# catid/siamese

Hardware: AMD Instinct MI355X
Metric: device-resident GB/s encode+decode, 1400B pkts @20% loss; % HBM peak (higher is better)
Workload: dtype u8

## Files before the change

### siamese_amd/csrc/decoder.cpp

```cpp
#include "decoder.h"
#include "frames.h"

#include <algorithm>
#include <atomic>
#include <cstdio>
#include <cstdlib>
#include <cstring>
#include <x86intrin.h>

namespace sgpu {

namespace {

inline unsigned popcount_range(uint64_t bits, unsigned begin, unsigned end)
{
    if (begin >= end)
        return 0;
    uint64_t mask = (end >= 64 ? ~0ULL : ((1ULL << end) - 1)) & ~((1ULL << begin) - 1);
    return (unsigned)__builtin_popcountll(bits & mask);
}

inline unsigned first_clear(uint64_t bits, unsigned from)
{
    if (from >= 64)
// ... 2222 lines not shown

bool DecoderCore::pivoted_ge(unsigned pivot)
{
    const unsigned columns = matCols_;
    const unsigned rows = matRows_;
    unsigned j = pivot + 1;
    bool resume = true;
    for (; pivot < columns; ++pivot) {
        if (!resume)
            j = pivot;
        resume = false;
        bool found = false;
        for (; j < rows; ++j) {
            const unsigned rj = pivots_[j];
            const uint8_t* ge = mrow(rj);
            const uint8_t val = ge[pivot];
            if (val == 0)
                continue;
            if (pivot != j)
                std::swap(pivots_[pivot], pivots_[j]);
            rows_[rj].used = true;
            const unsigned end = rows_[rj].columnCount;
            if (pivot >= columns - 1)
                return true;
            for (unsigned k = pivot + 1; k < rows; ++k) {
                const unsigned rk = pivots_[k];
                if (eliminate_row(ge, mrow(rk), pivot, end, val) && rows_[rk].columnCount < end)
                    rows_[rk].columnCount = end;
            }
            found = true;
            break;
        }
        if (!found) {
            geResume_ = pivot;
            return false;
        }
    }
    return true;
}


bool DecoderCore::eliminate_original_data()
{
    ++scanEpoch_;
    const unsigned rows = region_.recoveryCount;
    bool haveRun = false;
    unsigned runStart = 0, runCount = 0, runEnd = 0, runBytes = 0, runSumStart = 0;
    uint32_t fresh = 0;
    WinEntry sums[kRowSums];
    uint32_t clip[kRowSums];
    uint32_t present = 0;
    bool tableStale = true;
    uint64_t tableVersion = 0;
    for (unsigned ri = 0; ri < rows; ++ri) {
        if (!rows_[ri].used)
            continue;
        RecPacket* rec = rows_[ri].rec;
        const RowMeta m = rec->meta;
        const unsigned es = rec->elementStart;
        const unsigned ee = rec->elementEnd;
        const unsigned rb = rec->bytes;

        if (m.sumCount <= kCauchyThreshold) {
            prog_.lc_begin(rec->buf.addr(), rb, rb);
            for (unsigned j = es; j < ee; ++j) {
                const DecSlot& o = slot(j);
                if (o.bytes == 0)
                    continue;
                const uint8_t y = m.row == 0 ? 1 : cauchy_element(m.row - 1, o.column % kCauchyMaxColumns);
                prog_.lc_term(o.buf.addr(), std::min(o.bytes, rb), y);
                account_elim(std::min(o.bytes, rb));
            }
            prog_.lc_end();
            continue;
        }

        const bool sameRun = haveRun && m.columnStart == runStart && m.sumCount == runCount &&
                             ee == runEnd && rb == runBytes && recoveredColumns_.empty();
        unsigned sumElementStart = column_to_element(m.columnStart);
        if (!sameRun) {
            if (m.columnStart != sumColumnStart_ || m.sumCount < sumColumnCount_) {
                if (sumElementStart >= count_)
                    return false;
                reset_sums(sumElementStart);
                sumColumnStart_ = m.columnStart;
            } else {
                if (sumElementStart >= count_)
                    sumElementStart = 0;
                if (!start_sums(sumElementStart, rb))
                    return false;
            }
            sumColumnCount_ = m.sumCount;
            haveRun = true;
            runStart = m.columnStart;
            runCount = m.sumCount;
            runEnd = ee;
            runBytes = rb;
            fresh = 0;
            tableStale = true;
            runSumStart = sumElementStart;
        }

        windowLo_ = std::min(es, runSumStart);
        const RowSelect& sel = row_select(m.row);
        const uint32_t want = sel.mask[0] | sel.mask[1];
        uint32_t need = want & ~fresh;
        if (need)
            tableStale = true;
        for (; need; need &= need - 1) {
            const unsigned k = (unsigned)__builtin_ctz(need);
            if (get_sum(k / kSums, k % kSums, ee).bytes > 0)
                materialize(k / kSums, k % kSums);
        }
        fresh |= want;
        if (tableStale) {
            tableStale = false;
            tableVersion = Program::next_table_version();
            present = 0;
            for (unsigned k = 0; k < kRowSums; ++k) {
                const DevSum& d = sum(k / kSums, k % kSums).d;
                WinEntry& t = sums[k];
                t.src = d.buf.addr();
                t.len = d.bytes;
                t.column = 0;
                if (d.bytes > 0)
                    present |= 1u << k;
                clip[k] = std::min(d.bytes, rb);
            }
        }
        uint64_t opBytes = rb;
        for (uint32_t b = sel.mask[0] & present; b; b &= b - 1)
            opBytes += clip[__builtin_ctz(b)];
        for (uint32_t b = sel.mask[1] & present; b; b &= b - 1)
            opBytes += clip[__builtin_ctz(b)];
        const uint32_t mask[2] = {sel.mask[0] & present, sel.mask[1] & present};
        cover(windowLo_, ee);
        prog_.rows_row(sums, rec->buf.addr(), rb, rb, row_value(m.row), mask[0], mask[1], m.row,
                       m.ldpcCount, es, ee, nullptr, 0, tableVersion);
        account_elim(opBytes);
    }
    prog_.rows_seal();
    return !disabled_;
}


SiameseResult DecoderCore::solve_and_substitute()
{
    unsigned slot = 0;
    if (!solve_plan(0, &slot)) {
        disabled_ = true;
        return Siamese_Disabled;
    }
    return solve_publish(slot);
}

bool DecoderCore::solve_plan(uint32_t gateWord, unsigned* slotOut)
{
    const unsigned m = region_.lostCount;
    std::vector<RecPacket*>& pr = scratchRec_;
    std::vector<unsigned>& len = scratchLen_;
    pr.resize(m);
    len.resize(m);
    for (unsigned i = 0; i < m; ++i) {
        pr[i] = rows_[pivots_[i]].rec;
        len[i] = pr[i]->bytes;
    }
    SolveRow* desc = nullptr;
    uint8_t* coefOut = nullptr;
    prog_.solve_reserve(m, &desc, &coefOut);
    for (unsigned i = 0; i < m; ++i) {
        std::memset(&desc[i], 0, sizeof(SolveRow));
        desc[i].initBytes = len[i];
    }
    uint64_t lowerOpBytes = 0;
    bool equal = true;
    for (unsigned i = 1; i < m && equal; ++i)
        equal = len[i] == len[0];
    if (equal) {
        if (!gateWord) {
            uint64_t nz = 0;
            for (unsigned j = 1; j < m; ++j)
                nz += gf_count_nonzero(mrow(pivots_[j]), j);
            lowerOpBytes = nz * (m ? len[0] : 0);
        }
        for (unsigned i = 0; i + 1 < m; ++i)
            desc[i].lowerLen = len[i];
    } else {
        for (unsigned i = 0; i + 1 < m; ++i) {
            desc[i].lowerLen = len[i];
            for (unsigned j = i + 1; j < m; ++j) {
                if (mrow(pivots_[j])[i] == 0)
                    continue;
                lowerOpBytes += len[i];
// ... 536 lines not shown
```

### siamese_amd/csrc/encoder.cpp

```cpp
#include "encoder.h"
#include "frames.h"

#include <algorithm>
#include <atomic>
#include <cstdio>
#include <cstdlib>
#include <cstring>

namespace sgpu {

namespace {

constexpr unsigned kSlotCauses = 6;
const char* const kSlotCauseNames[kSlotCauses] = {"add", "length", "stride", "stamp", "arq", "other"};
struct SlotCounts
{
    const bool on = std::getenv("SIAMESE_AMD_SLOT_COUNTS") != nullptr;
    std::atomic<uint64_t> encoders{0}, uniform{0}, writes{0};
    std::atomic<uint64_t> demote[kSlotCauses] = {};
    ~SlotCounts()
    {
        if (!on)
            return;
        std::fprintf(stderr, "slot counts: encoders %llu enc_uniform %llu enc_slot_writes %llu",
// ... 879 lines not shown
    stats_[SiameseEncoderStats_RecoveryCount]++;
    stats_[SiameseEncoderStats_RecoveryBytes] += out.bytes;
}

SiameseResult EncoderCore::encode(EncodeOut& out)
{
    lastRowSiamese_ = false;
    if (dead())
        return Siamese_Disabled;
    if (count_ == 0) {
        out.bytes = 0;
        return Siamese_NeedMoreData;
    }
    if (firstUnremoved_ >= kRemoveThreshold)
        remove_elements();

    const unsigned inFlight = unacked();
    if (inFlight == 1)
        return single_row(out);

    const unsigned sumWidthBound = count_ - sumStart_ + sumErased_;
    if (sumEnd_ <= sumStart_ || sumWidthBound >= kMaxPacketsInFlight) {
        if (inFlight <= kCauchyThreshold)
            return cauchy_row(out);
        reset_sums(firstUnremoved_);
    } else if (inFlight <= kSumResetThreshold || sumWidthBound <= kCauchyThreshold) {
        sumEnd_ = sumStart_;
        return cauchy_row(out);
    }

    const unsigned row = nextRow_;
    if (++nextRow_ >= kRowValuePeriod)
        nextRow_ = 0;
    return siamese_row(out, row);
}

SiameseResult EncoderCore::encode_range(EncodeOut* out, unsigned count, unsigned* produced)
{
    for (DevBuf& b : recoveryHeld_)
        eng_->release(b);
    recoveryHeld_.clear();
    return encode_range_more(out, count, produced);
}

SiameseResult EncoderCore::encode_range_more(EncodeOut* out, unsigned count, unsigned* produced)
{
    *produced = 0;
    std::vector<DevBuf> held;
    held.swap(recoveryHeld_);
    SiameseResult r = Siamese_Success;
    bool siamese = false;
    uint64_t opAcc = 0, outAcc = 0;
    for (unsigned k = 0; k < count; ++k) {
        if (k > 0 || !held.empty() || *produced) {
            held.push_back(recovery_);
            recovery_ = DevBuf();
        }
        if (siamese) {
            if (dead()) {
                r = Siamese_Disabled;
                break;
            }
            const unsigned row = nextRow_;
            if (++nextRow_ >= kRowValuePeriod)
                nextRow_ = 0;
            recovery_ = eng_->alloc(longest_ + kMaxFooterBytes);
            if (!recovery_) {
                disabled_ = true;
                r = Siamese_Disabled;
                break;
            }
            uint64_t ob = 0;
            r = siamese_row_body(out[k], row, &ob);
            if (r != Siamese_Success)
                break;
            opAcc += ob;
            outAcc += out[k].bytes;
        } else {
            r = encode(out[k]);
            if (r != Siamese_Success)
                break;
            siamese = lastRowSiamese_;
        }
        ++*produced;
    }
    eng_->account(opAcc, outAcc);
    recoveryHeld_.swap(held);
    return r;
}

SiameseResult EncoderCore::single_row(EncodeOut& out)
{
    const SlotView o = peek(firstUnremoved_);
    if (!ensure_recovery(o.bytes + kMaxFooterBytes))
        return Siamese_Disabled;
    prog_.lc_begin(recovery_.addr(), o.bytes, 0);
    prog_.lc_term(o.addr(), o.bytes, 1);
    prog_.lc_end();
    write_length_prefix(o.bytes - o.header, out.head);
    RowMeta m;
    m.sumCount = 1;
    m.ldpcCount = 1;
    m.columnStart = o.column;
    m.row = 0;
    finish_row(out, m, o.bytes);
    return Siamese_Success;
// ... 70 lines not shown
        get_sum(k / kSums, k % kSums, count_);
        if (dead())
            return Siamese_Disabled;
    }
    staleSums_ &= ~want;
    if (sumTableStale_ || sumClipBytes_ != recoveryBytes) {
        sumTableStale_ = false;
        sumTableVersion_ = Program::next_table_version();
        sumPresent_ = 0;
        sumClipBytes_ = recoveryBytes;
        for (unsigned k = 0; k < kRowSums; ++k) {
            const DevSum& d = lanes_[k / kSums].sum[k % kSums];
            WinEntry& t = sumTable_[k];
            t.src = d.buf.addr();
            t.len = d.bytes;
            t.column = 0;
            if (d.bytes > 0)
                sumPresent_ |= 1u << k;
            sumClip_[k] = std::min(d.bytes, recoveryBytes);
        }
    }
    const uint32_t mask[2] = {sel.mask[0] & sumPresent_, sel.mask[1] & sumPresent_};
    uint64_t opBytes = recoveryBytes;
    for (unsigned h = 0; h < 2; ++h)
        for (uint32_t b = mask[h]; b; b &= b - 1)
            opBytes += sumClip_[__builtin_ctz(b)];
    sumEnd_ = count_;

    RowMeta m;
    m.sumCount = sumEnd_ - sumStart_ + sumErased_;
    m.ldpcCount = unacked();
    m.columnStart = sumColumnStart_;
    m.row = row;
    const unsigned footerBytes = write_footer(m, out.footer);

    const unsigned start = firstUnremoved_;
    const unsigned n = sumEnd_ - start;

    cover(std::min(start, sumStart_), sumEnd_);
    prog_.rows_row(sumTable_, recovery_.addr(), recoveryBytes, 0, row_value(row), mask[0], mask[1], row,
                   n, start, count_, out.footer, footerBytes, sumTableVersion_);

    out.meta = m;
    out.footerBytes = footerBytes;
    out.buf = recovery_;
    out.bytes = recoveryBytes + footerBytes;
    stats_[SiameseEncoderStats_RecoveryCount]++;
    stats_[SiameseEncoderStats_RecoveryBytes] += out.bytes;
    lastRowSiamese_ = true;
    *opBytesOut = opBytes;
    return Siamese_Success;
}

SiameseResult EncoderCore::stats(uint64_t* out, unsigned count)
{
    if (count > SiameseEncoderStats_Count)
        count = SiameseEncoderStats_Count;
    uint64_t mem = recovery_.cap;
    for (auto& sw : subwindows_) {
        mem += sw->slab.buf.cap;
        if (sw->clean)
            continue;
        for (EncSlot& s : sw->slot)
            if (!s.inSlab)
                mem += s.buf.cap;
    }
    for (Lane& l : lanes_)
        for (DevSum& s : l.sum)
            mem += s.buf.cap;
    stats_[SiameseEncoderStats_MemoryUsed] = mem;
    for (unsigned i = 0; i < count; ++i)
        out[i] = stats_[i];
    return Siamese_Success;
}

}
```

### siamese_amd/csrc/encoder.h

```cpp
#pragma once

#include "arq.h"
#include "codedef.h"
#include "engine.h"
#include "objpool.h"
#include "../../include/siamese.h"

#include <memory>
#include <vector>

namespace sgpu {

struct EncSlot
{
    DevBuf buf;
    bool inSlab = false;
    unsigned bytes = 0;
    unsigned column = 0;
    unsigned header = 0;
    uint32_t lastSend = 0;
    std::unique_ptr<std::vector<uint8_t>> hostp;
    std::vector<uint8_t>& host()
    {
        if (!hostp)
// ... 148 lines not shown
        }
        return v;
    }
    void demote(EncSubwindow* sw, DemoteCause cause);
    static uint64_t run_bits(unsigned bit, unsigned m) { return (m >= 64 ? ~0ull : (1ull << m) - 1) << bit; }
    bool uniform_takes(EncSubwindow* sw, unsigned element, unsigned m, unsigned need, unsigned h, unsigned column,
                       uint32_t stamp);
    void add_uniform(EncSubwindow* sw, unsigned element, unsigned m, unsigned need, unsigned h, unsigned bytes,
                     unsigned column, uint32_t stamp);
    void release_subwindow(EncSubwindow* sw);
#ifdef SGPU_SLOT_CHECK
    void slot_check(const EncSubwindow* sw, const char* where) const;
    struct AddExpect
    {
        unsigned nextColumn, longest, laneLongest[kLanes], count;
        uint32_t stale;
        uint64_t oc, ob;
        size_t subs;
    };
    AddExpect slot_check_add(EncSubwindow* sw, unsigned element, unsigned m, const unsigned* lens, unsigned fixedBytes,
                             uint32_t stamp);
    void slot_check_added(const AddExpect& x) const;
    [[noreturn]] static void slot_check_failed(const char* where, const char* what, unsigned bit);
#endif
    unsigned column_to_element(unsigned c) const { return column_sub(c, columnStart_); }
    unsigned element_to_column(unsigned e) const { return column_add(e, columnStart_); }
    unsigned next_lane_element(unsigned element, unsigned lane) const
    {
        unsigned e = element - (element % kLanes) + lane;
        return e < element ? e + kLanes : e;
    }
    unsigned unacked() const { return count_ - firstUnremoved_; }
    unsigned take_element();
    bool place(unsigned element, unsigned need);
    void fill_slot(EncSlot& s, unsigned column, unsigned header, unsigned dataBytes, uint32_t stamp);
    void release_slot(EncSlot& s)
    {
        if (!s.inSlab)
            eng_->release(s.buf);
        s.buf = DevBuf();
        s.inSlab = false;
    }
    void start_window(unsigned column);
    void reset_sums(unsigned elementStart);
    void remove_elements();
    DevSum& get_sum(unsigned lane, unsigned sumIndex, unsigned elementEnd);
    void cover(unsigned lo, unsigned hi);
    bool grow_sum(DevSum& s, unsigned bytes);

    SiameseResult single_row(EncodeOut& out);
    SiameseResult cauchy_row(EncodeOut& out);
    SiameseResult siamese_row(EncodeOut& out, unsigned row);
    SiameseResult siamese_row_body(EncodeOut& out, unsigned row, uint64_t* opBytes);
    bool ensure_recovery(unsigned bytes);
    void finish_row(EncodeOut& out, const RowMeta& meta, unsigned payloadBytes,
                    bool footerWritten = false);
    void update_rto();
    SiameseResult retransmit_slot(EncSlot& s, SiameseOriginalPacket& out);
    AckState ack_;

    Engine* eng_;
    Program prog_;
    bool mirror_;
    bool disabled_ = false;

    std::vector<EncSubwindowPtr> subwindows_;
    struct SubwindowTable
    {
        std::vector<EncSubwindowPtr> v;
        std::vector<DevBuf> held;
    };
    unsigned nextColumn_ = 0;
    unsigned count_ = 0;
    unsigned columnStart_ = 0;
    unsigned longest_ = 0;
    unsigned firstUnremoved_ = 0;
    unsigned sumStart_ = 0, sumEnd_ = 0, sumColumnStart_ = 0, sumErased_ = 0;

    struct Lane
    {
        unsigned next[kSums];
        DevSum sum[kSums];
        unsigned longest = 0;
    } lanes_[kLanes];

    static constexpr uint32_t kAllSums = (1u << kRowSums) - 1;
    uint32_t staleSums_ = kAllSums;
    WinEntry sumTable_[kRowSums];
    uint32_t sumPresent_ = 0;
    bool sumTableStale_ = true;
    uint64_t sumTableVersion_ = 0;
    uint32_t sumClip_[kRowSums] = {};
    unsigned sumClipBytes_ = ~0u;
    bool lastRowSiamese_ = false;

    DevBuf recovery_;
    std::vector<DevBuf> recoveryHeld_;
    unsigned nextRow_ = 0;
    unsigned nextParityColumn_ = 0;
    unsigned nextCauchyRow_ = 0;

    uint64_t stats_[SiameseEncoderStats_Count] = {};

    unsigned uniformEntered_ = 0, slotWrites_ = 0;
    unsigned demotions_[kDemoteCauses] = {};
};
// ... 3 lines not shown
```

### siamese_amd/csrc/engine.cpp

```cpp
#include "engine.h"

#include <pthread.h>
#include "backend.h"
#include "codedef.h"
#include "pool.h"

#include <algorithm>
#include <chrono>
#include <cmath>
#include <cstdio>
#include <cstddef>
#include <cstdlib>
#include <cstring>

#ifndef SGPU_EXEC_LPT
#define SGPU_EXEC_LPT 1
#endif
#ifndef SGPU_EXEC_GROUPS
#define SGPU_EXEC_GROUPS 256
#endif

namespace sgpu {

void EngineStats::add(const EngineStats& o)
// ... 56 lines not shown
    }
    return new ProgramBody;
}

void ProgramBody::put(ProgramBody* b)
{
    b->clear();
    std::lock_guard<std::mutex> g(g_bodyMu);
    if (g_bodies.size() < (1u << 15))
        g_bodies.push_back(b);
    else
        delete b;
}

void ProgramBody::clear()
{
    for (size_t k = 0; k < nsegs; ++k)
        segs[k].clear();
    nsegs = 0;
    resultWords = 0;
    nsolves = 0;
    nges = 0;
    callbacks.clear();
    keep.clear();
    rb.open = false;
    rb.win.clear();
    rb.updates.clear();
    rb.rows.clear();
    copies.clear();
    lcb.clear();
    ndeliver = 0;
    nframe = 0;
    frameLit.clear();
    frameLitRefs.clear();
    nrelay = 0;
    npackjob = npack = 0;
    nconcatjob = nconcat = 0;
    gateOpen = false;
}

void ProgramBody::new_segment()
{
    rows_close();
    if (nsegs == segs.size())
        segs.emplace_back();
    segs[nsegs++].clear();
}

void ProgramBody::rows_open(uint32_t base, bool keepWindow)
{
    rows_close();
    if (nsegs == 0)
        new_segment();
    rb.open = true;
    rb.haveSums = false;
    rb.sumsVersion = 0;
    rb.readMask = 0;
    rb.cutMax = 0;
    rb.versioned = false;
    if (!keepWindow) {
        rb.base = base;
        rb.win.clear();
    }
    rb.updates.clear();
    for (int& u : rb.updateOf)
        u = -1;
    rb.rows.clear();
    rb.maxExtent = 0;
}

namespace {
inline bool overlaps(uint64_t a, uint64_t an, uint64_t b, uint64_t bn) { return a < b + bn && b < a + an; }
inline uint64_t lane_span(uint32_t n) { return ((uint64_t)n + 15) & ~(uint64_t)15; }
}

void ProgramBody::lc_seal()
{
    if (lcb.items.empty())
        return;
    Segment& s = segs[nsegs - 1];
    if (lcb.items.size() == 1) {
        const LcItem& it = lcb.items[0];
        GfOp op;
        std::memset(&op, 0, sizeof(op));
        op.dst = it.dst;
        op.n = it.n;
        op.valid = it.valid;
        op.kind = OP_LINCOMB;
        op.mix = it.mixLit & 0xff;
        op.termBegin = (uint32_t)s.terms.size();
        op.termCount = it.termCount;
        s.ops.push_back(op);
        s.terms.insert(s.terms.end(), lcb.terms.begin(), lcb.terms.end());
        const uint32_t litLen = (it.mixLit >> 8) & 0xff;
        if (litLen) {
            GfOp lo;
            std::memset(&lo, 0, sizeof(lo));
            lo.dst = it.dst;
            lo.n = it.litOffset;
            lo.valid = litLen;
            lo.kind = OP_LITERAL;
            std::memcpy(lo.lit, it.lit, litLen);
            s.ops.push_back(lo);
        }
        lcb.clear();
        return;
    }
    const uint32_t itemWords = (uint32_t)lcb.items.size() * kLcWords;
    for (LcItem& it : lcb.items)
        it.termStart += itemWords;
    GfOp op;
    std::memset(&op, 0, sizeof(op));
    op.kind = OP_LINCOMBS;
    op.n = (uint32_t)lcb.items.size();
    op.termBegin = (uint32_t)(s.rowsData.size() / 16);
    op.termCount = itemWords + (uint32_t)lcb.terms.size();
    s.ops.push_back(op);
    const size_t at = s.rowsData.size();
    s.rowsData.resize(at + (size_t)op.termCount * 16);
    std::memcpy(s.rowsData.data() + at, lcb.items.data(), lcb.items.size() * sizeof(LcItem));
    std::memcpy(s.rowsData.data() + at + lcb.items.size() * sizeof(LcItem), lcb.terms.data(),
// ... 497 lines not shown
    return b.win.data() + (end - b.base);
}

void Program::rows_update(unsigned k, uint64_t dst, uint32_t n, uint32_t valid, unsigned s,
                          uint32_t fromElement, uint32_t toElement)
{
    ProgramBody::RowsBuild& b = b_->rb;
    if (b.readMask >> k & 1) {
        const WinEntry& seen = b.sums[k];
        if (seen.src != dst || valid < seen.len || toElement - fromElement > kVersionMaxSpan ||
            b.rows.size() >= kVersionRows)
            rows_open(b.base, true);
        else
            b.versioned = true;
    }
    const uint32_t from = fromElement - b.base, to = toElement - b.base;
    int& ui = b.updateOf[k];
    if (ui >= 0) {
        SumUpdate& u = b.updates[ui];
        const uint64_t d = ((uint64_t)u.dstHi << 32) | u.dstLo;
        if (d == dst && (u.to == from || from == to)) {
            if (from != to)
                u.to = to;
            if (n > u.n)
                u.n = n;
            if (n > b.maxExtent)
                b.maxExtent = n;
            return;
        }
        rows_open(b.base, true);
    }
    SumUpdate u;
    std::memset(&u, 0, sizeof(u));
    u.dstLo = (uint32_t)dst;
    u.dstHi = (uint32_t)(dst >> 32);
    u.n = n;
    u.valid = valid < n ? valid : n;
    u.s = s;
    u.from = from;
    u.to = to < from ? from : to;
    u.sum = k;
    b.updateOf[k] = (int)b.updates.size();
    b.updates.push_back(u);
    if (n > b.maxExtent)
        b.maxExtent = n;
}

uint64_t Program::next_table_version()
{
    static std::atomic<uint64_t> next{1};
    return next.fetch_add(1, std::memory_order_relaxed);
}

void Program::rows_row(const WinEntry* sums, uint64_t dst, uint32_t n, uint32_t valid, uint8_t mix,
                       uint32_t mask0, uint32_t mask1, unsigned row, uint32_t ldpcN,
                       uint32_t ldpcFirst, uint32_t cutoff, const uint8_t* lit, uint32_t litLen,
                       uint64_t sumsVersion)
{
    ProgramBody::RowsBuild& b = b_->rb;
    const bool unchanged = sumsVersion != 0 && b.haveSums && b.sumsVersion == sumsVersion;
    bool same = true;
    if (b.haveSums && !unchanged)
        for (uint32_t r = b.readMask; r; r &= r - 1) {
            const unsigned k = (unsigned)__builtin_ctz(r);
            if (std::memcmp(&b.sums[k], &sums[k], sizeof(WinEntry)) != 0) {
                same = false;
                break;
            }
        }
    if (!same || cutoff < b.cutMax || (b.versioned && b.rows.size() >= kVersionRows))
        rows_open(b.base, true);
    b.cutMax = std::max(b.cutMax, cutoff);
    if (!(unchanged && b.haveSums))
        std::memcpy(b.sums, sums, sizeof(b.sums));
    b.haveSums = true;
    b.sumsVersion = sumsVersion;
    RowItem r;
    std::memset(&r, 0, sizeof(r));
    r.dst = dst;
    r.n = n;
    r.valid = valid < n ? valid : n;
    r.mask0 = mask0 | (litLen << 24);
    r.mask1 = mask1 | ((uint32_t)mix << 24);
    r.row = row;
    r.ldpcN = ldpcN;
    r.ldpcOff = ldpcFirst - b.base;
    r.cutoff = cutoff - b.base;
    if (litLen)
        std::memcpy(r.lit, lit, litLen);
    b.rows.push_back(r);
    b.readMask |= mask0 | mask1;
    if (n + litLen > b.maxExtent)
        b.maxExtent = n + litLen;
}

void Program::copy(uint64_t dst, uint64_t src, uint32_t len)
{
    if (len == 0)
        return;
    touch();
    if (b_->copies.empty()) {
        b_->rows_close();
        if (b_->nsegs == 0)
            b_->new_segment();
    }
    CopyItem c;
    std::memset(&c, 0, sizeof(c));
    c.dst = dst;
    c.src = src;
    c.len = len;
    b_->copies.push_back(c);
    ProgramBody::Segment& g = b_->segs[b_->nsegs - 1];
    if (len > g.maxExtent)
        g.maxExtent = len;
}

void Program::deliver(uint64_t src, uint32_t cap, uint64_t dst, uint64_t lenOut, uint64_t stride)
{
    touch();
    DeliverItem it;
    it.src = src;
    it.dst = dst;
    it.lenOut = lenOut;
    it.cap = cap;
    it.stride16 = (uint32_t)(stride >> 4);
    if (b_->ndeliver == b_->delivers.size())
        b_->delivers.emplace_back();
    b_->delivers[b_->ndeliver++] = it;
}

void Program::frame(uint64_t src, uint32_t bytes, const uint8_t* hdr, uint32_t hdrLen, uint64_t dst,
                    uint64_t lenOut, uint64_t stride, uint32_t lenBase)
{
    touch();
    FrameItem it;
    it.src = src;
    it.dst = dst;
    it.lenOut = lenOut;
    it.bytes = bytes;
    it.stride16 = (uint32_t)(stride >> 4);
    std::memset(it.hdr, 0, sizeof(it.hdr));
    std::memcpy(it.hdr, hdr, hdrLen);
    it.hdrLen = (uint8_t)hdrLen;
    it.lenBase = lenBase;
    if (b_->nframe == b_->frames.size())
        b_->frames.emplace_back();
    b_->frames[b_->nframe++] = it;
}
// ... 252 lines not shown
        if (cls < depot_.size()) {
            auto& mags = depot_[cls];
            for (size_t k = mags.size(); k-- > 0;) {
                if (mags[k].ticket > done)
                    continue;
                list.swap(mags[k].bufs);
                mags.erase(mags.begin() + (long)k);
                if (!list.empty())
                    return true;
                break;
            }
        }
    }
    if (cap > kRegionBytes / 4) {
        uint8_t* p = carve_region(cap);
        if (!p)
            return false;
        list.push_back(p);
        return true;
    }
    const size_t want = std::max<size_t>(1, std::min<size_t>(kMagazine, kRefillBytes / cap));
    for (size_t k = 0; k < want; ++k) {
        if (s.bumpLeft < cap) {
            if (k > 0)
                break;
            uint8_t* r = carve_region(kRegionBytes);
            if (!r)
                return false;
            s.bump = r;
            s.bumpLeft = kRegionBytes;
        }
        list.push_back(s.bump);
        s.bump += cap;
        s.bumpLeft -= cap;
    }
    return true;
}

DevBuf Engine::alloc(uint32_t bytes)
{
    DevBuf b;
    const uint32_t cap = round_cap(bytes);
    Shard& s = shard();
    const size_t cls = cap_class(cap);
    if (cls >= s.freeLists.size())
        s.freeLists.resize(cls + 1);
    if (s.freeLists[cls].empty() && !refill(s, cls, cap))
        return DevBuf();
    b.ptr = s.freeLists[cls].back();
    s.freeLists[cls].pop_back();
    b.cap = cap;
    s.inUse += cap;
    return b;
}


DevBuf Engine::slab_slot(Slab& sl, unsigned bit, uint32_t need, bool* failed)
{
    *failed = false;
    if (!sl.buf) {
        static_assert(kSubwindow == 64, "slab_stride's slot count");
        const uint32_t stride = slab_stride(need);
        if (!stride)
            return DevBuf();
        sl.buf = alloc(stride * kSubwindow);
        if (!sl.buf) {
            *failed = true;
            return DevBuf();
        }
        sl.stride = stride;
        sl.used = 0;
    }
    if (need > sl.stride || (sl.used >> bit & 1u))
        return DevBuf();
    sl.used |= 1ull << bit;
    DevBuf b;
    b.ptr = sl.buf.ptr + (size_t)bit * sl.stride;
    b.cap = sl.stride;
    return b;
}

void Engine::release(DevBuf& b)
{
    if (b.ptr) {
        Shard& s = shard();
        const size_t cls = cap_class(b.cap);
        if (cls >= s.q.released.size())
            s.q.released.resize(cls + 1);
        s.q.released[cls].push_back(b.ptr);
        s.inUse -= b.cap;
    }
    b = DevBuf();
}

void Engine::download(void* hostDst, uint64_t devSrc, uint32_t bytes)
{
    if (bytes)
        shard().q.downloads.push_back(Shard::Download{hostDst, devSrc, bytes});
}

void Engine::stage_host_ingest(const DevBuf& dst, const void* data, uint32_t bytes,
                               const uint8_t* hdr, uint32_t hdrLen)
{
    Shard& s = shard();
    const size_t off = (s.q.hostStage.size() + 15) & ~(size_t)15;
    s.q.hostStage.resize(off + hdrLen + bytes);
// ... 1799 lines not shown
```

### siamese_amd/csrc/engine.h

```cpp
#pragma once

#include "ops.h"

#include <atomic>
#include <condition_variable>
#include <cstdint>
#include <cstdio>
#include <cstdlib>
#include <deque>
#include <functional>
#include <memory>
#include <mutex>
#include <pthread.h>
#include <shared_mutex>
#include <thread>
#include <vector>

namespace sgpu {

class InstanceLock
{
public:
    InstanceLock() = default;
    InstanceLock(const InstanceLock&) = delete;
// ... 147 lines not shown
using Completion = std::function<void(const uint32_t* results)>;

struct ProgramBody
{
    struct Segment
    {
        std::vector<GfOp> ops;
        std::vector<GfTerm> terms;
        std::vector<uint8_t> rowsData;
        uint32_t rowsWords = 0;
        uint32_t maxExtent = 0;
        struct Wide
        {
            uint32_t op;
            uint32_t entry;
            uint32_t n, row, N, off;
        };
        std::vector<Wide> wide;
        uint32_t wideItems = 0;
        uint64_t wideBytes = 0;
        struct Gate
        {
            uint32_t opBegin, opEnd, word;
        };
        std::vector<Gate> gates;
        void clear()
        {
            ops.clear();
            terms.clear();
            rowsData.clear();
            rowsWords = 0;
            maxExtent = 0;
            wide.clear();
            wideItems = 0;
            wideBytes = 0;
            gates.clear();
        }
    };
    struct RowsBuild
    {
        bool open = false;
        bool haveSums = false;
        uint64_t sumsVersion = 0;
        WinEntry sums[kRowSums];
        uint32_t readMask = 0;
        uint32_t cutMax = 0;
        bool versioned = false;
        uint32_t base = 0;
        std::vector<WinEntry> win;
        std::vector<SumUpdate> updates;
        int updateOf[kRowSums];
        std::vector<RowItem> rows;
        uint32_t maxExtent = 0;
    };
    struct PendingSolve
    {
        SolveDesc desc;
        std::vector<SolveRow> rows;
        std::vector<uint8_t> coef;
        mutable uint32_t asmRow = 0, asmCoef = 0;
    };
    struct PendingGe
    {
        uint16_t rows = 0, cols = 0;
        uint32_t pickLen = 0;
        uint32_t result = 0;
        bool chained = false;
        uint32_t solve = ~0u;
        std::vector<uint8_t> in;
    };

    int group = 0;
    uint32_t resultWords = 0;
    size_t nsegs = 0;
    std::vector<Segment> segs;
    std::vector<PendingSolve> solves;
    size_t nsolves = 0;
    std::vector<PendingGe> ges;
    uint32_t nges = 0;
    uint32_t ndeliver = 0;
    uint32_t nframe = 0;
    uint32_t nrelay = 0;
    std::vector<Completion> callbacks;
    std::vector<std::shared_ptr<void>> keep;
    RowsBuild rb;
    bool gateOpen = false;
    size_t gateSeg = 0;
    uint32_t gateOp = 0, gateWord = 0;
    std::vector<CopyItem> copies;
    struct LcBuild
    {
        std::vector<LcItem> items;
        std::vector<GfTerm> terms;
        struct Span
        {
            uint64_t lo, hi;
        };
        std::vector<Span> writes, reads;
        void clear()
        {
            items.clear();
            terms.clear();
            writes.clear();
            reads.clear();
        }
    } lcb;
// ... 53 lines not shown
            len = op.n;
        if (len == 0 || coeff == 0)
            return;
        GfTerm t;
        t.src = src;
        t.len = len;
        t.coeff = coeff;
        t.acc = acc;
        t.pad = 0;
        s.terms.push_back(t);
        ++op.termCount;
    }
    void lc_end();

    void add_mem(uint64_t dst, uint64_t src, uint32_t n);
    void muladd_mem(uint64_t dst, uint8_t y, uint64_t src, uint32_t n);
    void mul_mem(uint64_t dst, uint64_t src, uint8_t y, uint32_t n);
    void zero(uint64_t dst, uint32_t n);

    void literal(uint64_t dst, uint32_t offset, const uint8_t* bytes, uint32_t len);

    void ingest_host(const DevBuf& dst, const void* data, uint32_t bytes, const uint8_t* hdr,
                     uint32_t hdrLen);
    void ingest_device(const DevBuf& dst, uint64_t src, uint32_t bytes, const uint8_t* hdr,
                       uint32_t hdrLen);
    void ingest_run(uint64_t dst, uint32_t dstStride, uint64_t src, uint32_t srcStride, uint32_t count,
                    uint32_t bytes, const uint8_t* hdr, uint32_t hdrLen);

    uint32_t solve(const std::vector<SolveRow>& rows, const uint8_t* coef, uint32_t maxBytes);
    void solve_reserve(unsigned m, SolveRow** rows, uint8_t** coef);
    uint32_t solve_commit(uint32_t maxBytes, uint32_t gateWord = 0);

    uint8_t* ge_job(unsigned rows, unsigned cols, unsigned pickLen, uint32_t* resultWord, bool chained = false);
    void gate_begin(uint32_t word);
    uint32_t gate_end();

    void on_complete(Completion fn);
    void on_complete(std::shared_ptr<void> keep, Completion fn);
    void drop_callbacks()
    {
        if (b_) {
            b_->callbacks.clear();
            b_->keep.clear();
        }
    }

    WinEntry* rows_window(uint32_t lo, uint32_t hi, uint32_t* from);
    void rows_update(unsigned sumIndex, uint64_t dst, uint32_t n, uint32_t valid, unsigned s,
                     uint32_t fromElement, uint32_t toElement);
    void rows_row(const WinEntry* sums, uint64_t dst, uint32_t n, uint32_t valid, uint8_t mix,
                  uint32_t mask0, uint32_t mask1, unsigned row, uint32_t ldpcN,
                  uint32_t ldpcFirst, uint32_t cutoff, const uint8_t* lit = nullptr, uint32_t litLen = 0,
                  uint64_t sumsVersion = 0);
    static uint64_t next_table_version();
    void rows_seal()
    {
        if (b_)
            b_->rows_close();
    }

    void copy(uint64_t dst, uint64_t src, uint32_t len);

    void deliver(uint64_t src, uint32_t cap, uint64_t dst, uint64_t lenOut, uint64_t stride);

    void frame(uint64_t src, uint32_t bytes, const uint8_t* hdr, uint32_t hdrLen, uint64_t dst, uint64_t lenOut,
               uint64_t stride, uint32_t lenBase = 0);
    void frame_literal(const uint8_t* data, uint32_t bytes, const uint8_t* hdr, uint32_t hdrLen, uint64_t dst,
                       uint64_t lenOut, uint64_t stride);

    void relay(uint64_t src, uint32_t cap, uint32_t flow, uint32_t packetNum, uint64_t dst, uint64_t lenOut,
               uint64_t stride);

    void pack(const PackItem* items, uint32_t count, uint64_t rows, uint64_t stride, uint32_t maxRows, uint64_t lens,
              uint64_t info);

    void concat(const ConcatItem* items, uint32_t count, uint32_t total, uint64_t dst, uint32_t capacity,
                uint64_t offsets, uint64_t info);

    bool empty() const { return !b_ || b_->empty(); }

private:
    friend class Engine;
    void touch()
    {
        if (!shard_)
            attach();
    }
    void attach();
    void rows_open(uint32_t base, bool keepWindow) { b_->rows_open(base, keepWindow); }

    Engine* eng_;
    int group_;
    Shard* shard_ = nullptr;
    ProgramBody* b_ = nullptr;
};

struct EngineStats
{
    uint64_t flushes = 0, launches = 0, ops = 0, terms = 0, solves = 0, ingests = 0;
    uint64_t uploadBytes = 0;
    uint64_t refOpBytes = 0, outBytes = 0;
    uint64_t solveBytes = 0;
    uint64_t ldpcBytes = 0;
    uint64_t assembleNs = 0, waitNs = 0, completeNs = 0, reclaimNs = 0;
    uint64_t execLaunches = 0;
    uint64_t execUniqueBytes = 0;
    uint64_t geJobs = 0, geChained = 0, geRetried = 0;
    uint64_t geChainedWide = 0;
    uint64_t delivers = 0;
    uint64_t frames = 0;
    uint64_t scans = 0;
    uint64_t relays = 0;

    void add(const EngineStats& o);
};

class Engine
{
public:
    static Engine* global();
    ~Engine();

    bool init(int device, const char** err);
    bool ready() const { return ready_; }

    DevBuf alloc(uint32_t bytes);
    void release(DevBuf& b);
    DevBuf slab_slot(Slab& sl, unsigned bit, uint32_t need, bool* failed);
    void slab_release(Slab& sl)
    {
        release(sl.buf);
        sl.stride = 0;
        sl.used = 0;
    }
    uint64_t bytes_in_use() const;
    uint64_t arena_bytes() const { return arenaBytes_.load(std::memory_order_relaxed); }
    bool reserve(size_t bytes);

    void download(void* hostDst, uint64_t devSrc, uint32_t bytes);

    uint64_t enqueue();
    bool wait(uint64_t ticket);
    bool done(uint64_t ticket)
    {
        std::lock_guard<std::mutex> g(qMu_);
        return doneTicket_ >= ticket;
    }
    uint64_t last_ticket() const { return nextTicket_.load(std::memory_order_acquire); }
    bool flush();
    bool sync() { return wait(nextTicket_.load(std::memory_order_acquire)); }
    bool flush_and_sync(InstanceLock* detach = nullptr);
    bool failed() const { return failed_.load(std::memory_order_relaxed); }
    bool pending() const;

    bool gather(unsigned count, const void* const* srcs, const unsigned* bytes, void* hostOut);
    bool gather_completed(unsigned count, const void* const* srcs, const unsigned* bytes, void* pinnedOut);
    int64_t gather_async(unsigned count, const void* const* srcs, const unsigned* bytes, void* pinnedOut);
    int64_t gather_async_framed(unsigned count, const void* const* srcs, const unsigned* bytes,
                                const uint8_t* hdrs, const unsigned* hdrLens, void* pinnedOut);
    int64_t scan_rows_async(const void* rows, uint64_t stride, const uint32_t* lens, unsigned count,
                            void* pinnedOut)
    {
        return rows_async(rows, stride, lens, count, 0, pinnedOut);
    }
    int64_t walk_rows_async(const void* rows, uint64_t stride, const uint32_t* lens, unsigned count,
                            unsigned maxFrames, void* pinnedOut)
    {
        return rows_async(rows, stride, lens, count, maxFrames, pinnedOut);
    }
    int64_t duplex_rows_async(const void* rows, uint64_t stride, const uint32_t* lens, unsigned count,
                              unsigned maxFrames, unsigned ackSlots, unsigned ackBytes, void* pinnedOut)
    {
        return rows_async(rows, stride, lens, count, maxFrames, pinnedOut, ackSlots, ackBytes);
    }
    int64_t dense_rows_async(const void* rows, uint64_t stride, const uint32_t* lens, unsigned count,
                             unsigned maxFrames, unsigned maxRecords, void* pinnedOut)
    {
        return rows_async(rows, stride, lens, count, maxFrames, pinnedOut, 0, 0, maxRecords);
    }
// ... 191 lines not shown
```

Baseline: 4238.

## Batch consecutive Siamese recovery rows into single row-run submissions

```diff
diff --git a/siamese_amd/csrc/decoder.cpp b/siamese_amd/csrc/decoder.cpp
--- a/siamese_amd/csrc/decoder.cpp
+++ b/siamese_amd/csrc/decoder.cpp
@@ -2298,9 +2298,34 @@
     uint32_t present = 0;
     bool tableStale = true;
     uint64_t tableVersion = 0;
+    thread_local std::vector<Program::RowSpec> pend;
+    pend.clear();
+    uint64_t pendBytes = 0;
+    bool afterSiamese = false;
+    unsigned runEs = 0, runLdpc = 0;
+    auto flush_run = [&] {
+        if (pend.empty())
+            return;
+        Program::RowRun run;
+        run.sums = sums;
+        run.n = runBytes;
+        run.valid = runBytes;
+        run.ldpcN = runLdpc;
+        run.ldpcFirst = runEs;
+        run.cutoff = runEnd;
+        run.sumsVersion = tableVersion;
+        cover(windowLo_, runEnd);
+        prog_.rows_run(run, pend.data(), (unsigned)pend.size());
+        account_elim(pendBytes);
+        pend.clear();
+        pendBytes = 0;
+    };
     for (unsigned ri = 0; ri < rows; ++ri) {
-        if (!rows_[ri].used)
+        if (!rows_[ri].used) {
+            flush_run();
+            afterSiamese = false;
             continue;
+        }
         RecPacket* rec = rows_[ri].rec;
         const RowMeta m = rec->meta;
         const unsigned es = rec->elementStart;
@@ -2308,6 +2333,8 @@
         const unsigned rb = rec->bytes;
 
         if (m.sumCount <= kCauchyThreshold) {
+            flush_run();
+            afterSiamese = false;
             prog_.lc_begin(rec->buf.addr(), rb, rb);
             for (unsigned j = es; j < ee; ++j) {
                 const DecSlot& o = slot(j);
@@ -2323,6 +2350,25 @@
 
         const bool sameRun = haveRun && m.columnStart == runStart && m.sumCount == runCount &&
                              ee == runEnd && rb == runBytes && recoveredColumns_.empty();
+        const RowSelect& sel = row_select(m.row);
+        const uint32_t want = sel.mask[0] | sel.mask[1];
+        if (sameRun && afterSiamese && es == runEs && m.ldpcCount == runLdpc && !tableStale && !(want & ~fresh)) {
+            const uint32_t mask[2] = {sel.mask[0] & present, sel.mask[1] & present};
+            pendBytes += rb;
+            for (unsigned h = 0; h < 2; ++h)
+                for (uint32_t b = mask[h]; b; b &= b - 1)
+                    pendBytes += clip[__builtin_ctz(b)];
+            Program::RowSpec s;
+            std::memset(&s, 0, sizeof(s));
+            s.dst = rec->buf.addr();
+            s.row = m.row;
+            s.mask0 = mask[0];
+            s.mask1 = mask[1];
+            s.mix = row_value(m.row);
+            pend.push_back(s);
+            continue;
+        }
+        flush_run();
         unsigned sumElementStart = column_to_element(m.columnStart);
         if (!sameRun) {
             if (m.columnStart != sumColumnStart_ || m.sumCount < sumColumnCount_) {
@@ -2348,8 +2394,6 @@
         }
 
         windowLo_ = std::min(es, runSumStart);
-        const RowSelect& sel = row_select(m.row);
-        const uint32_t want = sel.mask[0] | sel.mask[1];
         uint32_t need = want & ~fresh;
         if (need)
             tableStale = true;
@@ -2384,7 +2428,11 @@
         prog_.rows_row(sums, rec->buf.addr(), rb, rb, row_value(m.row), mask[0], mask[1], m.row,
                        m.ldpcCount, es, ee, nullptr, 0, tableVersion);
         account_elim(opBytes);
-    }
+        afterSiamese = true;
+        runEs = es;
+        runLdpc = m.ldpcCount;
+    }
+    flush_run();
     prog_.rows_seal();
     return !disabled_;
 }
diff --git a/siamese_amd/csrc/encoder.cpp b/siamese_amd/csrc/encoder.cpp
--- a/siamese_amd/csrc/encoder.cpp
+++ b/siamese_amd/csrc/encoder.cpp
@@ -955,6 +955,19 @@
     bool siamese = false;
     uint64_t opAcc = 0, outAcc = 0;
     for (unsigned k = 0; k < count; ++k) {
+        if (siamese) {
+            const unsigned len = run_rows(count - k);
+            if (len > 1) {
+                const unsigned made = siamese_run(out + k, len, held, &opAcc, &outAcc);
+                *produced += made;
+                if (made < len) {
+                    r = Siamese_Disabled;
+                    break;
+                }
+                k += len - 1;
+                continue;
+            }
+        }
         if (k > 0 || !held.empty() || *produced) {
             held.push_back(recovery_);
             recovery_ = DevBuf();
@@ -1131,6 +1144,110 @@
     return Siamese_Success;
 }
 
+unsigned EncoderCore::run_rows(unsigned most) const
+{
+    if (sumTableStale_ || sumClipBytes_ != longest_)
+        return 0;
+    if (!staleSums_)
+        return most;
+    unsigned len = 0;
+    for (unsigned row = nextRow_; len < most; ++len) {
+        const RowSelect& sel = row_select(row);
+        if ((sel.mask[0] | sel.mask[1]) & staleSums_)
+            break;
+        if (++row >= kRowValuePeriod)
+            row = 0;
+    }
+    return len;
+}
+
+unsigned EncoderCore::siamese_run(EncodeOut* out, unsigned count, std::vector<DevBuf>& held, uint64_t* opAcc,
+                                  uint64_t* outAcc)
+{
+    if (dead()) {
+        held.push_back(recovery_);
+        recovery_ = DevBuf();
+        return 0;
+    }
+    thread_local std::vector<DevBuf> runBufs_;
+    thread_local std::vector<Program::RowSpec> runSpec_;
+    runBufs_.resize(count);
+    const unsigned got = eng_->alloc_run(longest_ + kMaxFooterBytes, runBufs_.data(), count);
+
+    const unsigned recoveryBytes = longest_;
+    RowMeta m;
+    m.sumCount = count_ - sumStart_ + sumErased_;
+    m.ldpcCount = unacked();
+    m.columnStart = sumColumnStart_;
+    m.row = 0;
+    uint8_t footer[kMaxFooterBytes] = {};
+    const unsigned footerBytes = write_footer(m, footer);
+    const bool footerRow = m.sumCount > 1;
+    const unsigned start = firstUnremoved_;
+    const unsigned bytes = recoveryBytes + footerBytes;
+
+    if (got) {
+        sumEnd_ = count_;
+        cover(std::min(start, sumStart_), sumEnd_);
+        runSpec_.resize(got);
+    }
+    uint64_t opBytes = 0;
+    for (unsigned k = 0; k < got; ++k) {
+        held.push_back(recovery_);
+        recovery_ = runBufs_[k];
+        const unsigned row = nextRow_;
+        if (++nextRow_ >= kRowValuePeriod)
+            nextRow_ = 0;
+        const RowSelect& sel = row_select(row);
+        const uint32_t mask[2] = {sel.mask[0] & sumPresent_, sel.mask[1] & sumPresent_};
+        opBytes += recoveryBytes;
+        for (unsigned h = 0; h < 2; ++h)
+            for (uint32_t b = mask[h]; b; b &= b - 1)
+                opBytes += sumClip_[__builtin_ctz(b)];
+        if (footerRow)
+            footer[0] = (uint8_t)row;
+        Program::RowSpec& s = runSpec_[k];
+        s.dst = recovery_.addr();
+        s.row = row;
+        s.mask0 = mask[0];
+        s.mask1 = mask[1];
+        s.mix = row_value(row);
+        s.litLen = (uint8_t)footerBytes;
+        std::memcpy(s.lit, footer, sizeof(s.lit));
+        EncodeOut& o = out[k];
+        m.row = row;
+        o.meta = m;
+        std::memcpy(o.footer, footer, footerBytes);
+        o.footerBytes = footerBytes;
+        o.buf = recovery_;
+        o.bytes = bytes;
+    }
+    if (got) {
+        Program::RowRun run;
+        run.sums = sumTable_;
+        run.n = recoveryBytes;
+        run.valid = 0;
+        run.ldpcN = sumEnd_ - start;
+        run.ldpcFirst = start;
+        run.cutoff = count_;
+        run.sumsVersion = sumTableVersion_;
+        prog_.rows_run(run, runSpec_.data(), got);
+        stats_[SiameseEncoderStats_RecoveryCount] += got;
+        stats_[SiameseEncoderStats_RecoveryBytes] += (uint64_t)got * bytes;
+        lastRowSiamese_ = true;
+        *opAcc += opBytes;
+        *outAcc += (uint64_t)got * bytes;
+    }
+    if (got < count) {
+        held.push_back(recovery_);
+        recovery_ = DevBuf();
+        if (++nextRow_ >= kRowValuePeriod)
+            nextRow_ = 0;
+        disabled_ = true;
+    }
+    return got;
+}
+
 SiameseResult EncoderCore::stats(uint64_t* out, unsigned count)
 {
     if (count > SiameseEncoderStats_Count)
diff --git a/siamese_amd/csrc/encoder.h b/siamese_amd/csrc/encoder.h
--- a/siamese_amd/csrc/encoder.h
+++ b/siamese_amd/csrc/encoder.h
@@ -224,6 +224,9 @@
     SiameseResult cauchy_row(EncodeOut& out);
     SiameseResult siamese_row(EncodeOut& out, unsigned row);
     SiameseResult siamese_row_body(EncodeOut& out, unsigned row, uint64_t* opBytes);
+    unsigned run_rows(unsigned most) const;
+    unsigned siamese_run(EncodeOut* out, unsigned count, std::vector<DevBuf>& held, uint64_t* opAcc,
+                         uint64_t* outAcc);
     bool ensure_recovery(unsigned bytes);
     void finish_row(EncodeOut& out, const RowMeta& meta, unsigned payloadBytes,
                     bool footerWritten = false);
diff --git a/siamese_amd/csrc/engine.cpp b/siamese_amd/csrc/engine.cpp
--- a/siamese_amd/csrc/engine.cpp
+++ b/siamese_amd/csrc/engine.cpp
@@ -132,21 +132,26 @@
     rows_close();
     if (nsegs == 0)
         new_segment();
-    rb.open = true;
-    rb.haveSums = false;
-    rb.sumsVersion = 0;
-    rb.readMask = 0;
-    rb.cutMax = 0;
-    rb.versioned = false;
+    rb.restart(base, keepWindow);
+}
+
+void ProgramBody::RowsBuild::restart(uint32_t newBase, bool keepWindow)
+{
+    open = true;
+    haveSums = false;
+    sumsVersion = 0;
+    readMask = 0;
+    cutMax = 0;
+    versioned = false;
     if (!keepWindow) {
-        rb.base = base;
-        rb.win.clear();
-    }
-    rb.updates.clear();
-    for (int& u : rb.updateOf)
+        base = newBase;
+        win.clear();
+    }
+    updates.clear();
+    for (int& u : updateOf)
         u = -1;
-    rb.rows.clear();
-    rb.maxExtent = 0;
+    rows.clear();
+    maxExtent = 0;
 }
 
 namespace {
@@ -750,12 +755,13 @@
     return next.fetch_add(1, std::memory_order_relaxed);
 }
 
-void Program::rows_row(const WinEntry* sums, uint64_t dst, uint32_t n, uint32_t valid, uint8_t mix,
-                       uint32_t mask0, uint32_t mask1, unsigned row, uint32_t ldpcN,
-                       uint32_t ldpcFirst, uint32_t cutoff, const uint8_t* lit, uint32_t litLen,
-                       uint64_t sumsVersion)
-{
-    ProgramBody::RowsBuild& b = b_->rb;
+namespace {
+
+template <class Open>
+inline void row_into(ProgramBody::RowsBuild& b, Open&& open, const WinEntry* sums, uint64_t dst, uint32_t n,
+                     uint32_t valid, uint8_t mix, uint32_t mask0, uint32_t mask1, unsigned row, uint32_t ldpcN,
+                     uint32_t ldpcFirst, uint32_t cutoff, const uint8_t* lit, uint32_t litLen, uint64_t sumsVersion)
+{
     const bool unchanged = sumsVersion != 0 && b.haveSums && b.sumsVersion == sumsVersion;
     bool same = true;
     if (b.haveSums && !unchanged)
@@ -767,7 +773,7 @@
             }
         }
     if (!same || cutoff < b.cutMax || (b.versioned && b.rows.size() >= kVersionRows))
-        rows_open(b.base, true);
+        open();
     b.cutMax = std::max(b.cutMax, cutoff);
     if (!(unchanged && b.haveSums))
         std::memcpy(b.sums, sums, sizeof(b.sums));
@@ -792,6 +798,150 @@
         b.maxExtent = n + litLen;
 }
 
+#ifdef SGPU_ROWRUN_CHECK
+struct RowRunCheck
+{
+    struct Seen
+    {
+        bool haveSums, versioned;
+        WinEntry sums[kRowSums];
+        uint32_t readMask, cutMax, maxExtent;
+        std::vector<RowItem> rows;
+    };
+    static Seen see(const ProgramBody::RowsBuild& b)
+    {
+        Seen s;
+        s.haveSums = b.haveSums;
+        s.versioned = b.versioned;
+        std::memcpy(s.sums, b.sums, sizeof(s.sums));
+        s.readMask = b.readMask;
+        s.cutMax = b.cutMax;
+        s.maxExtent = b.maxExtent;
+        s.rows = b.rows;
+        return s;
+    }
+    static bool equal(const Seen& a, const Seen& b)
+    {
+        return a.haveSums == b.haveSums && a.versioned == b.versioned &&
+               (!a.haveSums || std::memcmp(a.sums, b.sums, sizeof(a.sums)) == 0) && a.readMask == b.readMask &&
+               a.cutMax == b.cutMax && a.maxExtent == b.maxExtent && a.rows.size() == b.rows.size() &&
+               (a.rows.empty() || std::memcmp(a.rows.data(), b.rows.data(), a.rows.size() * sizeof(RowItem)) == 0);
+    }
+    ProgramBody::RowsBuild shadow;
+    std::vector<Seen> want, got;
+
+    RowRunCheck(const ProgramBody::RowsBuild& b, const Program::RowRun& run, const Program::RowSpec* rows,
+                unsigned count)
+        : shadow(b)
+    {
+        for (unsigned k = 0; k < count; ++k) {
+            const Program::RowSpec& s = rows[k];
+            row_into(
+                shadow,
+                [&] {
+                    want.push_back(see(shadow));
+                    shadow.restart(shadow.base, true);
+                },
+                run.sums, s.dst, run.n, run.valid, s.mix, s.mask0, s.mask1, s.row, run.ldpcN, run.ldpcFirst,
+                run.cutoff, s.lit, s.litLen, run.sumsVersion);
+        }
+    }
+    void closing(const ProgramBody::RowsBuild& b) { got.push_back(see(b)); }
+    void done(const ProgramBody::RowsBuild& b)
+    {
+        want.push_back(see(shadow));
+        got.push_back(see(b));
+        bool ok = want.size() == got.size() && shadow.sumsVersion == b.sumsVersion && shadow.base == b.base;
+        for (size_t k = 0; ok && k < want.size(); ++k)
+            ok = equal(want[k], got[k]);
+        if (!ok) {
+            std::fprintf(stderr, "rows_run: the run differs from its rows emitted one by one (%zu / %zu batches)\n",
+                         got.size(), want.size());
+            std::abort();
+        }
+    }
+};
+#endif
+
+}
+
+void Program::rows_row(const WinEntry* sums, uint64_t dst, uint32_t n, uint32_t valid, uint8_t mix,
+                       uint32_t mask0, uint32_t mask1, unsigned row, uint32_t ldpcN,
+                       uint32_t ldpcFirst, uint32_t cutoff, const uint8_t* lit, uint32_t litLen,
+                       uint64_t sumsVersion)
+{
+    ProgramBody::RowsBuild& b = b_->rb;
+    row_into(b, [&] { rows_open(b.base, true); }, sums, dst, n, valid, mix, mask0, mask1, row, ldpcN, ldpcFirst,
+             cutoff, lit, litLen, sumsVersion);
+}
+
+void Program::rows_run(const RowRun& run, const RowSpec* rows, unsigned count)
+{
+    if (count == 0)
+        return;
+    ProgramBody::RowsBuild& b = b_->rb;
+#ifdef SGPU_ROWRUN_CHECK
+    RowRunCheck check(b, run, rows, count);
+#define ROWRUN_CLOSING() check.closing(b)
+#else
+#define ROWRUN_CLOSING() (void)0
+#endif
+    const bool unchanged = run.sumsVersion != 0 && b.haveSums && b.sumsVersion == run.sumsVersion;
+    bool same = true;
+    if (b.haveSums && !unchanged)
+        for (uint32_t r = b.readMask; r; r &= r - 1) {
+            const unsigned k = (unsigned)__builtin_ctz(r);
+            if (std::memcmp(&b.sums[k], &run.sums[k], sizeof(WinEntry)) != 0) {
+                same = false;
+                break;
+            }
+        }
+    bool fresh = !same || run.cutoff < b.cutMax || (b.versioned && b.rows.size() >= kVersionRows);
+    const uint32_t valid = run.valid < run.n ? run.valid : run.n;
+    for (unsigned k = 0; k < count;) {
+        if (fresh) {
+            ROWRUN_CLOSING();
+            rows_open(b.base, true);
+        }
+        b.cutMax = std::max(b.cutMax, run.cutoff);
+        if (!(unchanged && b.haveSums))
+            std::memcpy(b.sums, run.sums, sizeof(b.sums));
+        b.haveSums = true;
+        b.sumsVersion = run.sumsVersion;
+        unsigned take = count - k;
+        if (b.versioned)
+            take = std::min<unsigned>(take, kVersionRows - (unsigned)b.rows.size());
+        const size_t at = b.rows.size();
+        b.rows.resize(at + take);
+        RowItem* r = b.rows.data() + at;
+        const uint32_t ldpcOff = run.ldpcFirst - b.base, cutoff = run.cutoff - b.base;
+        uint32_t read = 0, litMax = 0;
+        for (const RowSpec *s = rows + k, *end = s + take; s < end; ++s, ++r) {
+            r->dst = s->dst;
+            r->n = run.n;
+            r->valid = valid;
+            r->mask0 = s->mask0 | ((uint32_t)s->litLen << 24);
+            r->mask1 = s->mask1 | ((uint32_t)s->mix << 24);
+            r->row = s->row;
+            r->ldpcN = run.ldpcN;
+            r->ldpcOff = ldpcOff;
+            r->cutoff = cutoff;
+            std::memcpy(r->lit, s->lit, sizeof(r->lit));
+            read |= s->mask0 | s->mask1;
+            litMax = std::max<uint32_t>(litMax, s->litLen);
+        }
+        b.readMask |= read;
+        if (run.n + litMax > b.maxExtent)
+            b.maxExtent = run.n + litMax;
+        k += take;
+        fresh = true;
+    }
+#undef ROWRUN_CLOSING
+#ifdef SGPU_ROWRUN_CHECK
+    check.done(b);
+#endif
+}
+
 void Program::copy(uint64_t dst, uint64_t src, uint32_t len)
 {
     if (len == 0)
@@ -1150,6 +1300,30 @@
     b.cap = cap;
     s.inUse += cap;
     return b;
+}
+
+unsigned Engine::alloc_run(uint32_t bytes, DevBuf* out, unsigned count)
+{
+    const uint32_t cap = round_cap(bytes);
+    Shard& s = shard();
+    const size_t cls = cap_class(cap);
+    if (cls >= s.freeLists.size())
+        s.freeLists.resize(cls + 1);
+    unsigned got = 0;
+    while (got < count) {
+        std::vector<uint8_t*>& list = s.freeLists[cls];
+        if (list.empty() && !refill(s, cls, cap))
+            break;
+        const size_t take = std::min<size_t>(count - got, list.size());
+        for (size_t k = 0; k < take; ++k) {
+            out[got].ptr = list[list.size() - 1 - k];
+            out[got].cap = cap;
+            ++got;
+        }
+        list.resize(list.size() - take);
+    }
+    s.inUse += (int64_t)cap * got;
+    return got;
 }
 
 
diff --git a/siamese_amd/csrc/engine.h b/siamese_amd/csrc/engine.h
--- a/siamese_amd/csrc/engine.h
+++ b/siamese_amd/csrc/engine.h
@@ -223,6 +223,7 @@
         int updateOf[kRowSums];
         std::vector<RowItem> rows;
         uint32_t maxExtent = 0;
+        void restart(uint32_t newBase, bool keepWindow);
     };
     struct PendingSolve
     {
@@ -382,6 +383,24 @@
                   uint32_t mask0, uint32_t mask1, unsigned row, uint32_t ldpcN,
                   uint32_t ldpcFirst, uint32_t cutoff, const uint8_t* lit = nullptr, uint32_t litLen = 0,
                   uint64_t sumsVersion = 0);
+    struct RowRun
+    {
+        const WinEntry* sums;
+        uint32_t n, valid;
+        uint32_t ldpcN, ldpcFirst;
+        uint32_t cutoff;
+        uint64_t sumsVersion;
+    };
+    struct RowSpec
+    {
+        uint64_t dst;
+        uint32_t row;
+        uint32_t mask0, mask1;
+        uint8_t mix;
+        uint8_t litLen;
+        uint8_t lit[8];
+    };
+    void rows_run(const RowRun& run, const RowSpec* rows, unsigned count);
     static uint64_t next_table_version();
     void rows_seal()
     {
@@ -455,6 +474,7 @@
     bool ready() const { return ready_; }
 
     DevBuf alloc(uint32_t bytes);
+    unsigned alloc_run(uint32_t bytes, DevBuf* out, unsigned count);
     void release(DevBuf& b);
     DevBuf slab_slot(Slab& sl, unsigned bit, uint32_t need, bool* failed);
     void slab_release(Slab& sl)
```

Result: slower. 4023 (-5.1%).
